# EryiXie/PlaneRecNet

Hardware: AMD Instinct MI355X
Metric: img/s fwd+bwd @480×640 ResNet101-DCN, 1/2/4/8 MI355X + roofline % (higher is better)
Workload: dtype f32 (tensors and accumulation fp32; plain GEMMs and the tap-walked 4x4/s2, 1x1/s2 and sub-pixel convolutions >= 300 tiles: 2xfp16-piece split MFMA, fp32 accumulate; fp32-only rate in fp32_only_run)

## Files before the change

planerecnet_amd/csrc/prn_dcn.hip:

```cpp
#include <stdlib.h>
#include "prn_common.h"

namespace {

struct Tap {
  int i00, i01, i10, i11;
  float w00, w01, w10, w11;
  float gy00, gy01, gy10, gy11, gx00, gx01, gx10, gx11;
  float mod;
  float sig;
  bool pass_y, pass_x;
};

struct OmView {
  const float* off; const float* msk;
  int64_t off_bs, msk_bs;
  float maxoff;
  int raw, pad;
};

__device__ __forceinline__ Tap make_tap(const OmView& v, int b, int k, int ho, int wo, int Ho, int Wo,
                                        int H, int W, int stride, bool need_grad) {
  Tap t;
  const size_t plane = (size_t)Ho * Wo, pix = (size_t)ho * Wo + wo;
  const float* ob = v.off + (size_t)b * v.off_bs;
  const float ry = ob[(2 * k) * plane + pix], rx = ob[(2 * k + 1) * plane + pix];
  float dy = ry, dx = rx;
  t.pass_y = t.pass_x = true;
  if (v.raw) {
    const float maxoff = v.maxoff;
    const float rm = ob[(18 + k) * plane + pix];
    dy = fminf(fmaxf(ry, -maxoff), maxoff); dx = fminf(fmaxf(rx, -maxoff), maxoff);
    t.pass_y = (ry >= -maxoff) && (ry <= maxoff);
    t.pass_x = (rx >= -maxoff) && (rx <= maxoff);
    t.sig = 1.f / (1.f + expf(-rm));
    t.mod = 2.f * t.sig;
  } else {
    t.sig = 0.f;
    t.mod = v.msk ? v.msk[(size_t)b * v.msk_bs + (size_t)k * plane + pix] : 1.f;
  }
  const int ki = k / 3, kj = k - ki * 3;
  const float y = (float)(ho * stride - v.pad + ki) + dy, x = (float)(wo * stride - v.pad + kj) + dx;
  const bool inside = (y > -1.f) && (y < (float)H) && (x > -1.f) && (x < (float)W);
  const float fy = floorf(y), fx = floorf(x);
  const int y0 = (int)fy, x0 = (int)fx, y1 = y0 + 1, x1 = x0 + 1;
  const float ly = y - fy, lx = x - fx, hy = 1.f - ly, hx = 1.f - lx;
  const bool vy0 = inside && y0 >= 0, vy1 = inside && y1 <= H - 1, vx0 = x0 >= 0, vx1 = x1 <= W - 1;
  const bool v00 = vy0 && vx0, v01 = vy0 && vx1, v10 = vy1 && vx0, v11 = vy1 && vx1;
  t.i00 = v00 ? y0 * W + x0 : 0; t.i01 = v01 ? y0 * W + x1 : 0;
  t.i10 = v10 ? y1 * W + x0 : 0; t.i11 = v11 ? y1 * W + x1 : 0;
  t.w00 = v00 ? hy * hx : 0.f; t.w01 = v01 ? hy * lx : 0.f;
  t.w10 = v10 ? ly * hx : 0.f; t.w11 = v11 ? ly * lx : 0.f;
  if (need_grad) {
    t.gy00 = v00 ? -hx : 0.f; t.gy01 = v01 ? -lx : 0.f; t.gy10 = v10 ? hx : 0.f; t.gy11 = v11 ? lx : 0.f;
    t.gx00 = v00 ? -hy : 0.f; t.gx01 = v01 ? hy : 0.f; t.gx10 = v10 ? -ly : 0.f; t.gx11 = v11 ? ly : 0.f;
  }
  return t;
}

__global__ __launch_bounds__(256) void dcn_sample_kernel(const float* __restrict__ x, OmView om,
                                                         float* __restrict__ cols, int B, int C, int H, int W, int Ho,
                                                         int Wo, int stride) {
  const int64_t gid = (int64_t)blockIdx.x * blockDim.x + threadIdx.x;
  const int64_t plane = (int64_t)Ho * Wo;
  if (gid >= (int64_t)B * 9 * plane) return;
  const int pix = gid % plane, k = (gid / plane) % 9, b = gid / (9 * plane);
  const int ho = pix / Wo, wo = pix - ho * Wo;
  const Tap t = make_tap(om, b, k, ho, wo, Ho, Wo, H, W, stride, false);
  const int cper = (C + gridDim.y - 1) / gridDim.y;
  const int c0 = blockIdx.y * cper, c1 = min(C, c0 + cper);
  const size_t HW = (size_t)H * W;
  const float* xp = x + ((size_t)b * C + c0) * HW;
  float* cp = cols + (((size_t)b * C + c0) * 9 + k) * plane + pix;
  constexpr int UN = 8;
  int c = c0;
  for (; c + UN <= c1; c += UN) {
    float a00[UN], a01[UN], a10[UN], a11[UN];
#pragma unroll
    for (int u = 0; u < UN; ++u) {
      const float* q = xp + (size_t)u * HW;
      a00[u] = q[t.i00]; a01[u] = q[t.i01]; a10[u] = q[t.i10]; a11[u] = q[t.i11];
    }
    __builtin_amdgcn_sched_barrier(0);
#pragma unroll
    for (int u = 0; u < UN; ++u) cp[(size_t)u * 9 * plane] = t.mod * (t.w00 * a00[u] + t.w01 * a01[u] + t.w10 * a10[u] + t.w11 * a11[u]);
    xp += (size_t)UN * HW;
    cp += (size_t)UN * 9 * plane;
  }
  for (; c < c1; ++c) {
    const float v = t.w00 * xp[t.i00] + t.w01 * xp[t.i01] + t.w10 * xp[t.i10] + t.w11 * xp[t.i11];
    *cp = t.mod * v;
    xp += HW;
    cp += 9 * plane;
  }
}

__global__ __launch_bounds__(256) void dcn_dom_partial_kernel(const float* __restrict__ x, OmView om,
                                                              const float* __restrict__ dcols, float* __restrict__ part, int B,
                                                              int C, int H, int W, int Ho, int Wo, int stride) {
  const int64_t gid = (int64_t)blockIdx.x * blockDim.x + threadIdx.x;
  const int64_t plane = (int64_t)Ho * Wo;
  if (gid >= (int64_t)B * 9 * plane) return;
  const int pix = gid % plane, k = (gid / plane) % 9, b = gid / (9 * plane);
  const int ho = pix / Wo, wo = pix - ho * Wo;
  const Tap t = make_tap(om, b, k, ho, wo, Ho, Wo, H, W, stride, true);
  const int cper = (C + gridDim.y - 1) / gridDim.y;
  const int c0 = blockIdx.y * cper, c1 = min(C, c0 + cper);
  const size_t HW = (size_t)H * W;
  const float* xp = x + ((size_t)b * C + c0) * HW;
  const float* dp = dcols + (((size_t)b * C + c0) * 9 + k) * plane + pix;
  float gy = 0.f, gx = 0.f, gm = 0.f;
  constexpr int UN = 8;
  int c = c0;
  for (; c + UN <= c1; c += UN) {
    float g[UN], a00[UN], a01[UN], a10[UN], a11[UN];
#pragma unroll
    for (int u = 0; u < UN; ++u) {
      const float* q = xp + (size_t)u * HW;
      g[u] = dp[(size_t)u * 9 * plane];
      a00[u] = q[t.i00]; a01[u] = q[t.i01]; a10[u] = q[t.i10]; a11[u] = q[t.i11];
    }
    __builtin_amdgcn_sched_barrier(0);
#pragma unroll
    for (int u = 0; u < UN; ++u) {
      gm += g[u] * (t.w00 * a00[u] + t.w01 * a01[u] + t.w10 * a10[u] + t.w11 * a11[u]);
      gy += g[u] * (t.gy00 * a00[u] + t.gy01 * a01[u] + t.gy10 * a10[u] + t.gy11 * a11[u]);
      gx += g[u] * (t.gx00 * a00[u] + t.gx01 * a01[u] + t.gx10 * a10[u] + t.gx11 * a11[u]);
    }
    xp += (size_t)UN * HW;
    dp += (size_t)UN * 9 * plane;
  }
  for (; c < c1; ++c) {
    const float g = *dp;
    const float x00 = xp[t.i00], x01 = xp[t.i01], x10 = xp[t.i10], x11 = xp[t.i11];
    gm += g * (t.w00 * x00 + t.w01 * x01 + t.w10 * x10 + t.w11 * x11);
    gy += g * (t.gy00 * x00 + t.gy01 * x01 + t.gy10 * x10 + t.gy11 * x11);
    gx += g * (t.gx00 * x00 + t.gx01 * x01 + t.gx10 * x10 + t.gx11 * x11);
    xp += HW;
    dp += 9 * plane;
  }
  float* ob = part + ((size_t)blockIdx.y * B + b) * 27 * plane + pix;
  ob[(2 * k) * plane] = t.pass_y ? gy * t.mod : 0.f;
  ob[(2 * k + 1) * plane] = t.pass_x ? gx * t.mod : 0.f;
  ob[(18 + k) * plane] = om.raw ? gm * 2.f * t.sig * (1.f - t.sig) : gm;
}

__global__ void dcn_dom_final_kernel(const float* __restrict__ part, float* __restrict__ d_off, float* __restrict__ d_msk, int64_t n, int G,
                                     int plane) {
  const int64_t i = (int64_t)blockIdx.x * blockDim.x + threadIdx.x;
  if (i >= n) return;
  float s = 0.f;
  for (int g = 0; g < G; ++g) s += part[(size_t)g * n + i];
  if (d_msk == nullptr) { d_off[i] = s; return; }
  const int64_t b = i / (27 * (int64_t)plane), r = i - b * 27 * (int64_t)plane;
  if (r < 18 * (int64_t)plane) d_off[b * 18 * plane + r] = s;
  else d_msk[b * 9 * plane + (r - 18 * (int64_t)plane)] = s;
}

struct CsrEntry { int src; float w; };

__device__ __forceinline__ bool csr_before(const CsrEntry& a, const CsrEntry& b) {
  return a.src < b.src || (a.src == b.src && __float_as_uint(a.w) < __float_as_uint(b.w));
}
__device__ __forceinline__ void csr_sort_bin(CsrEntry* __restrict__ e, int n) {
  if (n <= 8) {
    unsigned long long k[8];
    const unsigned long long* __restrict__ q = reinterpret_cast<const unsigned long long*>(e);
#pragma unroll
    for (int i = 0; i < 8; ++i) {
      const unsigned long long v = i < n ? q[i] : ~0ull;
      k[i] = i < n ? ((v << 32) | (v >> 32)) : ~0ull;
    }
#define PRN_CSR_CX(I, J) { const unsigned long long lo = k[I] < k[J] ? k[I] : k[J], hi = k[I] < k[J] ? k[J] : k[I]; k[I] = lo; k[J] = hi; }
    PRN_CSR_CX(0, 2) PRN_CSR_CX(1, 3) PRN_CSR_CX(4, 6) PRN_CSR_CX(5, 7) PRN_CSR_CX(0, 4) PRN_CSR_CX(1, 5) PRN_CSR_CX(2, 6) PRN_CSR_CX(3, 7)
    PRN_CSR_CX(0, 1) PRN_CSR_CX(2, 3) PRN_CSR_CX(4, 5) PRN_CSR_CX(6, 7) PRN_CSR_CX(2, 4) PRN_CSR_CX(3, 5) PRN_CSR_CX(1, 4) PRN_CSR_CX(3, 6)
    PRN_CSR_CX(1, 2) PRN_CSR_CX(3, 4) PRN_CSR_CX(5, 6)
#undef PRN_CSR_CX
    unsigned long long* __restrict__ o = reinterpret_cast<unsigned long long*>(e);
#pragma unroll
    for (int i = 0; i < 8; ++i)
      if (i < n) o[i] = (k[i] << 32) | (k[i] >> 32);
    return;
  }
  for (int i = 1; i < n; ++i) {
    const CsrEntry v = e[i];
    int j = i - 1;
    while (j >= 0 && csr_before(v, e[j])) { e[j + 1] = e[j]; --j; }
    e[j + 1] = v;
  }
}
__global__ __launch_bounds__(256) void dcn_csr_sort_kernel(const int* __restrict__ starts, const int* __restrict__ counts, CsrEntry* __restrict__ entries, int nbins) {
  const int bin = blockIdx.x * 256 + threadIdx.x;
  if (bin < nbins && counts[bin] > 1) csr_sort_bin(entries + starts[bin], counts[bin]);
}

__global__ __launch_bounds__(256) void dcn_csr_count_kernel(OmView om, int* __restrict__ counts, int B, int H, int W,
                                                            int Ho, int Wo, int stride) {
  const int64_t gid = (int64_t)blockIdx.x * blockDim.x + threadIdx.x;
  const int plane = Ho * Wo;
  if (gid >= (int64_t)B * 9 * plane) return;
  const int pix = gid % plane, k = (gid / plane) % 9, b = gid / (9 * plane);
  const int ho = pix / Wo, wo = pix - ho * Wo;
  const Tap t = make_tap(om, b, k, ho, wo, Ho, Wo, H, W, stride, false);
  int* cb = counts + (size_t)(b * 9 + k) * H * W;
  if (t.w00 != 0.f) atomicAdd(cb + t.i00, 1);
  if (t.w01 != 0.f) atomicAdd(cb + t.i01, 1);
  if (t.w10 != 0.f) atomicAdd(cb + t.i10, 1);
  if (t.w11 != 0.f) atomicAdd(cb + t.i11, 1);
}

constexpr int SCAN_PER_THREAD = 8, SCAN_PER_BLOCK = 256 * SCAN_PER_THREAD;

__device__ __forceinline__ int block_sum_256(int v, int* sm) {
  for (int o = 32; o > 0; o >>= 1) v += __shfl_down(v, o);
  if ((threadIdx.x & 63) == 0) sm[threadIdx.x >> 6] = v;
  __syncthreads();
  const int t = sm[0] + sm[1] + sm[2] + sm[3];
  __syncthreads();
  return t;
}

__global__ __launch_bounds__(256) void dcn_csr_block_sums_kernel(const int* __restrict__ counts, int* __restrict__ bsum, int n) {
  __shared__ int sm[4];
  const int base = blockIdx.x * SCAN_PER_BLOCK + threadIdx.x * SCAN_PER_THREAD;
  int v = 0;
#pragma unroll
  for (int i = 0; i < SCAN_PER_THREAD; ++i) v += (base + i < n) ? counts[base + i] : 0;
  const int t = block_sum_256(v, sm);
  if (threadIdx.x == 0) bsum[blockIdx.x] = t;
}

__global__ __launch_bounds__(256) void dcn_csr_scan_kernel(int* __restrict__ counts, int* __restrict__ starts, const int* __restrict__ bsum,
                                                           int n) {
  __shared__ int sm[4];
  __shared__ int wave_tot[4];
  int pre = 0;
  for (int i = threadIdx.x; i < (int)blockIdx.x; i += 256) pre += bsum[i];
  pre = block_sum_256(pre, sm);
  const int base = blockIdx.x * SCAN_PER_BLOCK + threadIdx.x * SCAN_PER_THREAD;
  int c[SCAN_PER_THREAD], mine = 0;
#pragma unroll
  for (int i = 0; i < SCAN_PER_THREAD; ++i) { c[i] = (base + i < n) ? counts[base + i] : 0; mine += c[i]; }
  const int lane = threadIdx.x & 63, wv = threadIdx.x >> 6;
  int incl = mine;
  for (int o = 1; o < 64; o <<= 1) { const int u = __shfl_up(incl, o); if (lane >= o) incl += u; }
  if (lane == 63) wave_tot[wv] = incl;
  __syncthreads();
  int off = pre + incl - mine;
  for (int w = 0; w < wv; ++w) off += wave_tot[w];
#pragma unroll
  for (int i = 0; i < SCAN_PER_THREAD; ++i)
    if (base + i < n) { starts[base + i] = off; off += c[i]; counts[base + i] = 0; }
}

__global__ __launch_bounds__(256) void dcn_csr_fill_kernel(OmView om, const int* __restrict__ starts, int* __restrict__ cursor,
                                                           CsrEntry* __restrict__ entries, int B, int H, int W, int Ho, int Wo, int stride) {
  const int64_t gid = (int64_t)blockIdx.x * blockDim.x + threadIdx.x;
  const int plane = Ho * Wo;
  if (gid >= (int64_t)B * 9 * plane) return;
  const int pix = gid % plane, k = (gid / plane) % 9, b = gid / (9 * plane);
  const int ho = pix / Wo, wo = pix - ho * Wo;
  const Tap t = make_tap(om, b, k, ho, wo, Ho, Wo, H, W, stride, false);
  const size_t bb = (size_t)(b * 9 + k) * H * W;
  const int src = k * plane + pix;
  auto put = [&](int idx, float w) {
    if (w != 0.f) {
      const int pos = starts[bb + idx] + atomicAdd(cursor + bb + idx, 1);
      entries[pos] = CsrEntry{src, w * t.mod};
    }
  };
  put(t.i00, t.w00); put(t.i01, t.w01); put(t.i10, t.w10); put(t.i11, t.w11);
}

constexpr int CSR1_THREADS = 1024;
constexpr int CSR1_MAX_BINS = 15360;
static_assert(CSR1_MAX_BINS * 4 + (CSR1_THREADS / 64) * 4 <= 64 * 1024, "the bins and the scan scratch of one tap plane must fit gfx950's 64 KB of LDS per workgroup");

__global__ __launch_bounds__(CSR1_THREADS) void dcn_csr_build_kernel(OmView om, int* __restrict__ starts, int* __restrict__ counts,
                                                                      CsrEntry* __restrict__ entries, int H, int W, int Ho, int Wo, int stride) {
  extern __shared__ int csr_bins[];
  __shared__ int wave_tot[CSR1_THREADS / 64];
  const int bk = blockIdx.x, b = bk / 9, k = bk - b * 9;
  const int HW = H * W, plane = Ho * Wo, tid = threadIdx.x;
  for (int i = tid; i < HW; i += CSR1_THREADS) csr_bins[i] = 0;
  __syncthreads();
  for (int p = tid; p < plane; p += CSR1_THREADS) {
    const int ho = p / Wo, wo = p - ho * Wo;
    const Tap t = make_tap(om, b, k, ho, wo, Ho, Wo, H, W, stride, false);
    if (t.w00 != 0.f) atomicAdd(csr_bins + t.i00, 1);
    if (t.w01 != 0.f) atomicAdd(csr_bins + t.i01, 1);
    if (t.w10 != 0.f) atomicAdd(csr_bins + t.i10, 1);
    if (t.w11 != 0.f) atomicAdd(csr_bins + t.i11, 1);
  }
  __syncthreads();
  const int per = (HW + CSR1_THREADS - 1) / CSR1_THREADS;
  const int b0 = tid * per, b1 = min(HW, b0 + per);
  int mine = 0;
  for (int i = b0; i < b1; ++i) mine += csr_bins[i];
  const int lane = tid & 63, wv = tid >> 6;
  int incl = mine;
  for (int o = 1; o < 64; o <<= 1) { const int u = __shfl_up(incl, o); if (lane >= o) incl += u; }
  if (lane == 63) wave_tot[wv] = incl;
  __syncthreads();
  int off = incl - mine;
  for (int w = 0; w < wv; ++w) off += wave_tot[w];
  const int seg = bk * 4 * plane;
  const size_t gb = (size_t)bk * HW;
  for (int i = b0; i < b1; ++i) {
    const int c = csr_bins[i];
    starts[gb + i] = seg + off;
    counts[gb + i] = c;
    csr_bins[i] = off;
    off += c;
  }
  __syncthreads();
  for (int p = tid; p < plane; p += CSR1_THREADS) {
    const int ho = p / Wo, wo = p - ho * Wo;
    const Tap t = make_tap(om, b, k, ho, wo, Ho, Wo, H, W, stride, false);
    const int src = k * plane + p;
    if (t.w00 != 0.f) entries[seg + atomicAdd(csr_bins + t.i00, 1)] = CsrEntry{src, t.w00 * t.mod};
    if (t.w01 != 0.f) entries[seg + atomicAdd(csr_bins + t.i01, 1)] = CsrEntry{src, t.w01 * t.mod};
    if (t.w10 != 0.f) entries[seg + atomicAdd(csr_bins + t.i10, 1)] = CsrEntry{src, t.w10 * t.mod};
    if (t.w11 != 0.f) entries[seg + atomicAdd(csr_bins + t.i11, 1)] = CsrEntry{src, t.w11 * t.mod};
  }
  __syncthreads();
  for (int i = b0; i < b1; ++i) {
    const int beg = i > 0 ? csr_bins[i - 1] : 0, n = csr_bins[i] - beg;
    if (n > 1) csr_sort_bin(entries + seg + beg, n);
  }
}

template <int CH>
__global__ __launch_bounds__(256) void dcn_dx_gather_kernel(const float* __restrict__ dcols, const int* __restrict__ starts,
                                                            const int* __restrict__ counts, const CsrEntry* __restrict__ entries,
                                                            float* __restrict__ dx, int C, int HW, int plane) {
  const int q = blockIdx.x * 256 + threadIdx.x;
  if (q >= HW) return;
  const int b = blockIdx.z, c0 = blockIdx.y * CH;
  const size_t cstride = (size_t)9 * plane;
  const float* __restrict__ dp = dcols + ((size_t)b * C + c0) * cstride;
  float acc[CH];
#pragma unroll
  for (int cc = 0; cc < CH; ++cc) acc[cc] = 0.f;
  int st[9], cn[9];
#pragma unroll
  for (int k = 0; k < 9; ++k) {
    const size_t bin = (size_t)(b * 9 + k) * HW + q;
    st[k] = starts[bin];
    cn[k] = counts[bin];
  }
#pragma unroll
  for (int k = 0; k < 9; ++k) {
    const int s = st[k], n = cn[k];
    CsrEntry nxt;
    nxt.src = 0; nxt.w = 0.f;
    if (n > 0) nxt = entries[s];
    for (int e = s; e < s + n; ++e) {
      const CsrEntry en = nxt;
      if (e + 1 < s + n) nxt = entries[e + 1];
#pragma unroll
      for (int cc = 0; cc < CH; ++cc) acc[cc] += en.w * dp[cc * cstride + en.src];
    }
  }
  float* out = dx + ((size_t)b * C + c0) * HW + q;
#pragma unroll
  for (int cc = 0; cc < CH; ++cc)
    if (c0 + cc < C) out[(size_t)cc * HW] = acc[cc];
}

}

static int channel_groups(int C, int64_t threads) {
  static const int forced = prn_env_int("PRN_DCN_GROUPS", 0);
  int g = forced > 0 ? forced : (int)(1 + (256 * 8 * 256) / (threads > 0 ? threads : 1));
  if (g > 16) g = 16;
  if (g > C) g = C;
  while (g < C && C % g) ++g;
  return g < 1 ? 1 : g;
}

namespace {
OmView raw_view(const float* om, int Ho, int Wo, float max_offset) {
  OmView v;
  v.off = om; v.msk = nullptr; v.off_bs = v.msk_bs = (int64_t)27 * Ho * Wo; v.maxoff = max_offset; v.raw = 1; v.pad = 1;
  return v;
}
OmView desc_view(const prn_dcn_desc* d, const float* offset, const float* mask) {
  if (d->raw) { OmView v = raw_view(offset, d->Ho, d->Wo, d->max_offset); v.pad = d->pad; return v; }
  OmView v;
  v.off = offset; v.msk = mask; v.off_bs = (int64_t)18 * d->Ho * d->Wo; v.msk_bs = (int64_t)9 * d->Ho * d->Wo; v.maxoff = 0.f; v.raw = 0; v.pad = d->pad;
  return v;
}
}

extern "C" int prn_dcn_sample(const float* x, const float* om, float* cols, int B, int C, int H, int W, int Ho, int Wo,
                              int stride, float max_offset, void* stream) {
  PRN_REQUIRE(x && om && cols && B > 0 && C > 0 && H > 0 && W > 0 && Ho > 0 && Wo > 0, "prn_dcn_sample: bad arguments");
  PRN_REQUIRE(Ho == (H + 2 - 3) / stride + 1 && Wo == (W + 2 - 3) / stride + 1, "prn_dcn_sample: output size mismatch");
  const int64_t n = (int64_t)B * 9 * Ho * Wo;
  hipLaunchKernelGGL(dcn_sample_kernel, dim3(cdiv(n, 256), channel_groups(C, n)), dim3(256), 0, (hipStream_t)stream, x, raw_view(om, Ho, Wo, max_offset),
                     cols, B, C, H, W, Ho, Wo, stride);
  PRN_CHECK_LAUNCH("prn_dcn_sample");
  return 0;
}

namespace {
struct BwdWs { int64_t part, counts, starts, bsum, entries, total; int nbins, nblocks; };
BwdWs bwd_ws_layout(int B, int C, int H, int W, int Ho, int Wo) {
  auto up = [](int64_t v) { return (v + 255) / 256 * 256; };
  BwdWs l;
  l.nbins = B * 9 * H * W;
  l.nblocks = cdiv(l.nbins, SCAN_PER_BLOCK);
  l.part = 0;
  l.counts = up((int64_t)channel_groups(C, (int64_t)B * 9 * Ho * Wo) * B * 27 * Ho * Wo * 4);
  l.starts = l.counts + up((int64_t)l.nbins * 4);
  l.bsum = l.starts + up((int64_t)l.nbins * 4);
  l.entries = l.bsum + up((int64_t)l.nblocks * 4);
  l.total = l.entries + (int64_t)B * 9 * Ho * Wo * 4 * sizeof(CsrEntry);
  return l;
}

int launch_dom(const float* x, const OmView& v, const float* dcols, float* d_off, float* d_msk, char* wsb, const BwdWs& l, int B, int C, int H, int W,
               int Ho, int Wo, int stride, hipStream_t st) {
  const int64_t n = (int64_t)B * 9 * Ho * Wo;
  const int G = channel_groups(C, n);
  hipLaunchKernelGGL(dcn_dom_partial_kernel, dim3(cdiv(n, 256), G), dim3(256), 0, st, x, v, dcols, (float*)(wsb + l.part), B, C, H, W, Ho, Wo, stride);
  PRN_CHECK_LAUNCH("dcn d_om partial");
  const int64_t nom = (int64_t)B * 27 * Ho * Wo;
  hipLaunchKernelGGL(dcn_dom_final_kernel, dim3(cdiv(nom, 256)), dim3(256), 0, st, (const float*)(wsb + l.part), d_off, d_msk, nom, G, Ho * Wo);
  PRN_CHECK_LAUNCH("dcn d_om final");
  return 0;
}

int launch_dx(const OmView& v, const float* dcols, float* dx, char* wsb, const BwdWs& l, int B, int C, int H, int W, int Ho, int Wo, int stride,
              hipStream_t st) {
  const int64_t n = (int64_t)B * 9 * Ho * Wo;
  int* counts = (int*)(wsb + l.counts);
  int* starts = (int*)(wsb + l.starts);
  int* bsum = (int*)(wsb + l.bsum);
  CsrEntry* entries = (CsrEntry*)(wsb + l.entries);
  static const int one = prn_env_int("PRN_DCN_CSR1", 1);
  if (one && H * W <= CSR1_MAX_BINS) {
    hipLaunchKernelGGL(dcn_csr_build_kernel, dim3(B * 9), dim3(CSR1_THREADS), (size_t)H * W * sizeof(int), st, v, starts, counts, entries, H, W, Ho, Wo, stride);
  } else {
    if (hipMemsetAsync(counts, 0, (size_t)l.nbins * 4, st) != hipSuccess) { prn_set_error("dcn d-input: memset failed"); return 1; }
    hipLaunchKernelGGL(dcn_csr_count_kernel, dim3(cdiv(n, 256)), dim3(256), 0, st, v, counts, B, H, W, Ho, Wo, stride);
    hipLaunchKernelGGL(dcn_csr_block_sums_kernel, dim3(l.nblocks), dim3(256), 0, st, (const int*)counts, bsum, l.nbins);
    hipLaunchKernelGGL(dcn_csr_scan_kernel, dim3(l.nblocks), dim3(256), 0, st, counts, starts, (const int*)bsum, l.nbins);
    hipLaunchKernelGGL(dcn_csr_fill_kernel, dim3(cdiv(n, 256)), dim3(256), 0, st, v, (const int*)starts, counts, entries, B, H, W, Ho, Wo, stride);
    hipLaunchKernelGGL(dcn_csr_sort_kernel, dim3(cdiv(l.nbins, 256)), dim3(256), 0, st, (const int*)starts, (const int*)counts, entries, (int)l.nbins);
  }
  PRN_CHECK_LAUNCH("dcn d-input csr");
  const int HW = H * W;
  const int64_t blocks8 = (int64_t)cdiv(HW, 256) * cdiv(C, 8) * B;
  if (blocks8 >= 1024)
    hipLaunchKernelGGL((dcn_dx_gather_kernel<8>), dim3(cdiv(HW, 256), cdiv(C, 8), B), dim3(256), 0, st, dcols, (const int*)starts, (const int*)counts,
                       (const CsrEntry*)entries, dx, C, HW, Ho * Wo);
  else
    hipLaunchKernelGGL((dcn_dx_gather_kernel<4>), dim3(cdiv(HW, 256), cdiv(C, 4), B), dim3(256), 0, st, dcols, (const int*)starts, (const int*)counts,
                       (const CsrEntry*)entries, dx, C, HW, Ho * Wo);
  PRN_CHECK_LAUNCH("dcn d-input gather");
  return 0;
}
}

extern "C" int64_t prn_dcn_sample_bwd_ws_bytes(int B, int C, int H, int W, int Ho, int Wo) {
  if (B <= 0 || C <= 0 || H <= 0 || W <= 0 || Ho <= 0 || Wo <= 0 || (int64_t)B * 9 * H * W >= (1LL << 31)) return -1;
  return bwd_ws_layout(B, C, H, W, Ho, Wo).total;
}

extern "C" int prn_dcn_sample_bwd(const float* x, const float* om, const float* dcols, float* dx, float* d_om, void* ws,
                                  int B, int C, int H, int W, int Ho, int Wo, int stride, float max_offset, void* stream) {
  PRN_REQUIRE(x && om && dcols && dx && d_om && ws && B > 0 && C > 0, "prn_dcn_sample_bwd: bad arguments");
  PRN_REQUIRE((int64_t)B * 9 * H * W < (1LL << 31) && (int64_t)B * 36 * Ho * Wo < (1LL << 31), "prn_dcn_sample_bwd: map too large");
  hipStream_t st = (hipStream_t)stream;
  const BwdWs l = bwd_ws_layout(B, C, H, W, Ho, Wo);
  const OmView v = raw_view(om, Ho, Wo, max_offset);
  if (int e = launch_dom(x, v, dcols, d_om, nullptr, (char*)ws, l, B, C, H, W, Ho, Wo, stride, st)) return e;
  return launch_dx(v, dcols, dx, (char*)ws, l, B, C, H, W, Ho, Wo, stride, st);
}

namespace {
struct DataWs { int64_t dcols, gemm, rest, total; prn_conv_desc g; };
int data_ws_layout(const prn_dcn_desc* d, DataWs& l) {
  auto up = [](int64_t v) { return (v + 255) / 256 * 256; };
  prn_conv_desc& g = l.g;
  g.B = d->B; g.C = d->M; g.H = d->Ho; g.W = d->Wo; g.M = d->C * 9; g.KH = g.KW = 1; g.stride = 1; g.pad = 0; g.Ho = d->Ho; g.Wo = d->Wo;
  g.in_mode = PRN_IN_ZERO; g.dil = 1; g.epilogue = PRN_EPI_NONE; g.ystride = 0; g.yH = g.yW = 0; g.reserved = 0;
  g.opts = d->opts;
  const int64_t gb = prn_conv2d_fwd_ws_bytes(&g);
  if (gb < 0) return 2;
  if ((int64_t)d->B * 9 * d->H * d->W >= (1LL << 31) || (int64_t)d->B * 36 * d->Ho * d->Wo >= (1LL << 31)) { prn_set_error("prn_dcnv2_bwd: map too large"); return 2; }
  l.dcols = 0;
  l.gemm = up((int64_t)d->B * d->C * 9 * d->Ho * d->Wo * 4);
  l.rest = l.gemm + up(gb);
  l.total = l.rest + bwd_ws_layout(d->B, d->C, d->H, d->W, d->Ho, d->Wo).total;
  return 0;
}
int check_dcn_desc(const prn_dcn_desc* d, const char* who) {
  PRN_REQUIRE(d != nullptr && d->B > 0 && d->C > 0 && d->H > 0 && d->W > 0 && d->M > 0 && d->Ho > 0 && d->Wo > 0 && d->stride > 0 && d->pad >= 0,
              "%s: bad descriptor", who);
  PRN_REQUIRE(d->Ho == (d->H + 2 * d->pad - 3) / d->stride + 1 && d->Wo == (d->W + 2 * d->pad - 3) / d->stride + 1, "%s: output size mismatch", who);
  return 0;
}
}

extern "C" int64_t prn_dcnv2_bwd_ws_bytes(const prn_dcn_desc* d) {
  if (check_dcn_desc(d, "prn_dcnv2_bwd_ws_bytes")) return -1;
  DataWs l;
  if (data_ws_layout(d, l)) return -1;
  return l.total;
}

extern "C" int prn_dcnv2_bwd_input(const prn_dcn_desc* d, const float* dy, const float* wt, const void* wt_images, const float* offset, const float* mask,
                                   float* dx, void* ws, void* stream) {
  return prn_dcnv2_bwd_input_phase(d, dy, wt, wt_images, offset, mask, dx, ws, stream, 0);
}

extern "C" int prn_dcnv2_bwd_input_phase(const prn_dcn_desc* d, const float* dy, const float* wt, const void* wt_images, const float* offset, const float* mask,
                                         float* dx, void* ws, void* stream, int phase) {
  if (int e = check_dcn_desc(d, "prn_dcnv2_bwd_input")) return e;
  PRN_REQUIRE(dy && wt && offset && ws, "prn_dcnv2_bwd_input: null tensor");
  PRN_REQUIRE(phase >= 0 && phase <= 3, "prn_dcnv2_bwd_input: bad phase");
  DataWs l;
  if (int e = data_ws_layout(d, l)) return e;
  char* wsb = (char*)ws;
  if (phase <= 2)
    if (int e = prn_conv2d_fwd_counted(&l.g, dy, wt, wt_images, nullptr, nullptr, (float*)(wsb + l.dcols), wsb + l.gemm, nullptr, stream, phase)) return e;
  if (dx == nullptr || phase == 1 || phase == 2) return 0;
  const BwdWs bl = bwd_ws_layout(d->B, d->C, d->H, d->W, d->Ho, d->Wo);
  return launch_dx(desc_view(d, offset, mask), (const float*)(wsb + l.dcols), dx, wsb + l.rest, bl, d->B, d->C, d->H, d->W, d->Ho, d->Wo, d->stride,
                   (hipStream_t)stream);
}

extern "C" int prn_dcnv2_bwd_offset_mask(const prn_dcn_desc* d, const float* x, const float* offset, const float* mask, float* d_offset, float* d_mask,
                                         void* ws, void* stream) {
  if (int e = check_dcn_desc(d, "prn_dcnv2_bwd_offset_mask")) return e;
  PRN_REQUIRE(x && offset && d_offset && ws, "prn_dcnv2_bwd_offset_mask: null tensor");
  PRN_REQUIRE(d->raw || d_mask != nullptr, "prn_dcnv2_bwd_offset_mask: d_mask required unless the descriptor is raw (then d_offset is the [B,27,Ho,Wo] gradient)");
  DataWs l;
  if (int e = data_ws_layout(d, l)) return e;
  char* wsb = (char*)ws;
  const BwdWs bl = bwd_ws_layout(d->B, d->C, d->H, d->W, d->Ho, d->Wo);
  return launch_dom(x, desc_view(d, offset, mask), (const float*)(wsb + l.dcols), d_offset, d->raw ? nullptr : d_mask, wsb + l.rest, bl, d->B, d->C, d->H,
                    d->W, d->Ho, d->Wo, d->stride, (hipStream_t)stream);
}
```

Baseline: 188.5.

## Use channel-innermost column layout for DCNv2 backward gather and offset-gradient kernels

Recasts the DCNv2 backward column GEMM so the gradient columns come out as [B*P, 9, C], with channels innermost. This needs transposes of dy, the weights and x. New kernels then read those columns with vectorized float4 channel loads: a CSR gather for dx, and an offset/mask gradient kernel that uses wave shuffles and so no longer needs the partial-sum buffer and final reduction pass. The aim is to replace strided, uncoalesced column accesses with contiguous ones. The cost is extra transpose passes and more workspace, and the path is on by default behind an env switch.

After: 186.2. 0.988x the previous value.

```diff
diff --git a/planerecnet_amd/csrc/prn_dcn.hip b/planerecnet_amd/csrc/prn_dcn.hip
--- a/planerecnet_amd/csrc/prn_dcn.hip
+++ b/planerecnet_amd/csrc/prn_dcn.hip
@@ -368,6 +368,180 @@
     if (c0 + cc < C) out[(size_t)cc * HW] = acc[cc];
 }
 
+
+
+__global__ __launch_bounds__(256) void dcn_transpose_kernel(const float* __restrict__ in, float* __restrict__ out, int R, int Cn, int64_t irs, int64_t ors,
+                                                            int64_t izs, int64_t ozs) {
+  __shared__ float tile[32][33];
+  const int tx = threadIdx.x & 31, ty = threadIdx.x >> 5;
+  const int c0 = blockIdx.x * 32, r0 = blockIdx.y * 32;
+  const float* ip = in + (size_t)blockIdx.z * izs;
+  float* op = out + (size_t)blockIdx.z * ozs;
+#pragma unroll
+  for (int i = 0; i < 4; ++i) {
+    const int r = r0 + ty + 8 * i, c = c0 + tx;
+    if (r < R && c < Cn) tile[ty + 8 * i][tx] = ip[(size_t)r * irs + c];
+  }
+  __syncthreads();
+#pragma unroll
+  for (int i = 0; i < 4; ++i) {
+    const int c = c0 + ty + 8 * i, r = r0 + tx;
+    if (r < R && c < Cn) op[(size_t)c * ors + r] = tile[tx][ty + 8 * i];
+  }
+}
+
+template <bool VEC>
+__device__ __forceinline__ float4 load4(const float* __restrict__ v, int c, int C) {
+  if constexpr (VEC) {
+    return c < C ? *reinterpret_cast<const float4*>(v + c) : make_float4(0.f, 0.f, 0.f, 0.f);
+  } else {
+    float4 r;
+    r.x = c < C ? v[c] : 0.f; r.y = c + 1 < C ? v[c + 1] : 0.f; r.z = c + 2 < C ? v[c + 2] : 0.f; r.w = c + 3 < C ? v[c + 3] : 0.f;
+    return r;
+  }
+}
+
+constexpr int DXQ = 16;
+template <int GS, bool VEC>
+__global__ __launch_bounds__(DXQ * GS) void dcn_dx_cl_kernel(const float* __restrict__ G, const int* __restrict__ starts, const int* __restrict__ counts,
+                                                              const CsrEntry* __restrict__ entries, float* __restrict__ dx, int C, int HW, int plane) {
+  __shared__ float tile[4 * GS][DXQ + 1];
+  const int tid = threadIdx.x, grp = tid / GS, gl = tid % GS, lane = tid & 63, gbase = lane - gl;
+  const int b = blockIdx.z, cbase = blockIdx.y * 4 * GS, c = cbase + 4 * gl;
+  const int q = blockIdx.x * DXQ + grp;
+  const bool live = q < HW;
+  const float* __restrict__ Gb = G + (size_t)b * plane * 9 * C;
+  int st = 0, cn = 0;
+  if (live && gl < 9) {
+    const size_t bin = (size_t)(b * 9 + gl) * HW + q;
+    st = starts[bin]; cn = counts[bin];
+  }
+  int pre[10];
+  pre[0] = 0;
+#pragma unroll
+  for (int k = 0; k < 9; ++k) pre[k + 1] = pre[k] + __shfl(cn, gbase + k);
+  int stk[9];
+#pragma unroll
+  for (int k = 0; k < 9; ++k) stk[k] = __shfl(st, gbase + k);
+  const int T = pre[9];
+  float4 acc = make_float4(0.f, 0.f, 0.f, 0.f);
+  for (int t0 = 0; __any(t0 < T); t0 += GS) {
+    const int t = t0 + gl;
+    int off = 0;
+    float wgt = 0.f;
+    if (t < T) {
+      int k = 0;
+#pragma unroll
+      for (int j = 1; j < 9; ++j) k += (t >= pre[j]) ? 1 : 0;
+      int s = 0, p0 = 0;
+#pragma unroll
+      for (int j = 0; j < 9; ++j) { s = (j == k) ? stk[j] : s; p0 = (j == k) ? pre[j] : p0; }
+      const CsrEntry en = entries[s + (t - p0)];
+      off = ((en.src - k * plane) * 9 + k) * C;
+      wgt = en.w;
+    }
+    const int nround = min(GS, T - t0);
+    constexpr int UN = 8;
+    for (int e = 0; __any(e < nround); e += UN) {
+      float4 g[UN];
+      float w[UN];
+#pragma unroll
+      for (int u = 0; u < UN; ++u) {
+        const int o = __shfl(off, gbase + ((e + u) & (GS - 1)));
+        const float ww = __shfl(wgt, gbase + ((e + u) & (GS - 1)));
+        w[u] = (e + u < nround) ? ww : 0.f;
+        g[u] = load4<VEC>(Gb + ((e + u < nround) ? o : 0), c, C);
+      }
+      __builtin_amdgcn_sched_barrier(0);
+#pragma unroll
+      for (int u = 0; u < UN; ++u) { acc.x += w[u] * g[u].x; acc.y += w[u] * g[u].y; acc.z += w[u] * g[u].z; acc.w += w[u] * g[u].w; }
+    }
+  }
+  tile[4 * gl + 0][grp] = acc.x; tile[4 * gl + 1][grp] = acc.y; tile[4 * gl + 2][grp] = acc.z; tile[4 * gl + 3][grp] = acc.w;
+  __syncthreads();
+  const int q0 = blockIdx.x * DXQ;
+#pragma unroll
+  for (int i = 0; i < 4; ++i) {
+    const int idx = tid + i * DXQ * GS, cc = idx / DXQ, qi = idx % DXQ;
+    if (cbase + cc < C && q0 + qi < HW) dx[((size_t)b * C + cbase + cc) * HW + q0 + qi] = tile[cc][qi];
+  }
+}
+
+template <int GS, bool VEC>
+__global__ __launch_bounds__(256) void dcn_dom_cl_kernel(const float* __restrict__ xT, OmView om, const float* __restrict__ G, float* __restrict__ d_off,
+                                                         float* __restrict__ d_msk, int B, int C, int H, int W, int Ho, int Wo, int stride) {
+  const int tid = threadIdx.x, gl = tid % GS, lane = tid & 63, gbase = lane - gl;
+  const int plane = Ho * Wo;
+  const int64_t n = (int64_t)blockIdx.x * (256 / GS) + tid / GS;
+  const bool live = n < (int64_t)B * plane;
+  const int b = live ? (int)(n / plane) : 0, p = live ? (int)(n - (int64_t)b * plane) : 0;
+  const int ho = p / Wo, wo = p - ho * Wo;
+  const int myk = gl < 9 ? gl : 8;
+  const Tap t = make_tap(om, b, myk, ho, wo, Ho, Wo, H, W, stride, true);
+  const int j00 = (t.gy00 != 0.f || t.gx00 != 0.f) ? t.i00 * C : -1, j01 = (t.gy01 != 0.f || t.gx01 != 0.f) ? t.i01 * C : -1;
+  const int j10 = (t.gy10 != 0.f || t.gx10 != 0.f) ? t.i10 * C : -1, j11 = (t.gy11 != 0.f || t.gx11 != 0.f) ? t.i11 * C : -1;
+  const float* __restrict__ xb = xT + (size_t)b * H * W * C;
+  const float* __restrict__ gp = G + ((size_t)b * plane + p) * 9 * C;
+  float S0 = 0.f, S1 = 0.f, S2 = 0.f, S3 = 0.f;
+  constexpr int UT = 3;
+  for (int kb = 0; kb < 9; kb += UT) {
+    int o[UT][4];
+    float a[UT][4];
+#pragma unroll
+    for (int u = 0; u < UT; ++u) {
+      o[u][0] = __shfl(j00, gbase + kb + u); o[u][1] = __shfl(j01, gbase + kb + u);
+      o[u][2] = __shfl(j10, gbase + kb + u); o[u][3] = __shfl(j11, gbase + kb + u);
+      a[u][0] = a[u][1] = a[u][2] = a[u][3] = 0.f;
+    }
+    for (int c = 4 * gl; __any(c < C); c += 4 * GS) {
+      float4 g[UT], xv[UT][4];
+#pragma unroll
+      for (int u = 0; u < UT; ++u) {
+        g[u] = load4<VEC>(gp + (size_t)(kb + u) * C, c, C);
+#pragma unroll
+        for (int j = 0; j < 4; ++j) xv[u][j] = load4<VEC>(xb + (o[u][j] < 0 ? 0 : o[u][j]), c, C);
+      }
+      __builtin_amdgcn_sched_barrier(0);
+#pragma unroll
+      for (int u = 0; u < UT; ++u)
+#pragma unroll
+        for (int j = 0; j < 4; ++j) {
+          const float d = g[u].x * xv[u][j].x + g[u].y * xv[u][j].y + g[u].z * xv[u][j].z + g[u].w * xv[u][j].w;
+          a[u][j] += o[u][j] < 0 ? 0.f : d;
+        }
+    }
+#pragma unroll
+    for (int u = 0; u < UT; ++u) {
+      const bool h1 = (gl & 1) != 0, h2 = (gl & 2) != 0;
+      float k0 = h1 ? a[u][2] : a[u][0], k1 = h1 ? a[u][3] : a[u][1];
+      const float s0 = h1 ? a[u][0] : a[u][2], s1 = h1 ? a[u][1] : a[u][3];
+      k0 += __shfl_xor(s0, 1); k1 += __shfl_xor(s1, 1);
+      float kk = h2 ? k1 : k0;
+      const float ss = h2 ? k0 : k1;
+      kk += __shfl_xor(ss, 2);
+#pragma unroll
+      for (int w = 4; w < GS; w <<= 1) kk += __shfl_xor(kk, w);
+      const float r0 = __shfl(kk, gbase + 0), r1 = __shfl(kk, gbase + 2), r2 = __shfl(kk, gbase + 1), r3 = __shfl(kk, gbase + 3);
+      if (gl == kb + u) { S0 = r0; S1 = r1; S2 = r2; S3 = r3; }
+    }
+  }
+  if (!live || gl >= 9) return;
+  const float gm = t.w00 * S0 + t.w01 * S1 + t.w10 * S2 + t.w11 * S3;
+  const float gy = t.gy00 * S0 + t.gy01 * S1 + t.gy10 * S2 + t.gy11 * S3;
+  const float gx = t.gx00 * S0 + t.gx01 * S1 + t.gx10 * S2 + t.gx11 * S3;
+  const float vy = t.pass_y ? gy * t.mod : 0.f, vx = t.pass_x ? gx * t.mod : 0.f;
+  const float vm = om.raw ? gm * 2.f * t.sig * (1.f - t.sig) : gm;
+  const int k = gl;
+  if (d_msk == nullptr) {
+    float* ob = d_off + (size_t)b * 27 * plane + p;
+    ob[(size_t)(2 * k) * plane] = vy; ob[(size_t)(2 * k + 1) * plane] = vx; ob[(size_t)(18 + k) * plane] = vm;
+  } else {
+    float* ob = d_off + (size_t)b * 18 * plane + p;
+    ob[(size_t)(2 * k) * plane] = vy; ob[(size_t)(2 * k + 1) * plane] = vx;
+    d_msk[((size_t)b * 9 + k) * plane + p] = vm;
+  }
+}
+
 }
 
 static int channel_groups(int C, int64_t threads) {
@@ -406,13 +580,17 @@
 
 namespace {
 struct BwdWs { int64_t part, counts, starts, bsum, entries, total; int nbins, nblocks; };
-BwdWs bwd_ws_layout(int B, int C, int H, int W, int Ho, int Wo) {
+bool bwd_cl() {
+  static const int on = prn_env_int("PRN_DCN_BWD_CL", 1);
+  return on != 0;
+}
+BwdWs bwd_ws_layout(int B, int C, int H, int W, int Ho, int Wo, bool with_part = true) {
   auto up = [](int64_t v) { return (v + 255) / 256 * 256; };
   BwdWs l;
   l.nbins = B * 9 * H * W;
   l.nblocks = cdiv(l.nbins, SCAN_PER_BLOCK);
   l.part = 0;
-  l.counts = up((int64_t)channel_groups(C, (int64_t)B * 9 * Ho * Wo) * B * 27 * Ho * Wo * 4);
+  l.counts = with_part ? up((int64_t)channel_groups(C, (int64_t)B * 9 * Ho * Wo) * B * 27 * Ho * Wo * 4) : 0;
   l.starts = l.counts + up((int64_t)l.nbins * 4);
   l.bsum = l.starts + up((int64_t)l.nbins * 4);
   l.entries = l.bsum + up((int64_t)l.nblocks * 4);
@@ -433,7 +611,7 @@
 }
 
 int launch_dx(const OmView& v, const float* dcols, float* dx, char* wsb, const BwdWs& l, int B, int C, int H, int W, int Ho, int Wo, int stride,
-              hipStream_t st) {
+              hipStream_t st, bool cl = false) {
   const int64_t n = (int64_t)B * 9 * Ho * Wo;
   int* counts = (int*)(wsb + l.counts);
   int* starts = (int*)(wsb + l.starts);
@@ -452,6 +630,17 @@
   }
   PRN_CHECK_LAUNCH("dcn d-input csr");
   const int HW = H * W;
+  if (cl) {
+    const int lanes = cdiv(C < 256 ? C : 256, 4), gs = lanes <= 16 ? 16 : (lanes <= 32 ? 32 : 64);
+    const dim3 grid(cdiv(HW, DXQ), cdiv(C, 4 * gs), B);
+#define PRN_DX_CL(GS_, VEC_) hipLaunchKernelGGL((dcn_dx_cl_kernel<GS_, VEC_>), grid, dim3(DXQ * GS_), 0, st, dcols, (const int*)starts, (const int*)counts, \
+                                               (const CsrEntry*)entries, dx, C, HW, Ho * Wo)
+    if ((C & 3) == 0) { if (gs == 16) PRN_DX_CL(16, true); else if (gs == 32) PRN_DX_CL(32, true); else PRN_DX_CL(64, true); }
+    else { if (gs == 16) PRN_DX_CL(16, false); else if (gs == 32) PRN_DX_CL(32, false); else PRN_DX_CL(64, false); }
+#undef PRN_DX_CL
+    PRN_CHECK_LAUNCH("dcn d-input gather (channel-innermost)");
+    return 0;
+  }
   const int64_t blocks8 = (int64_t)cdiv(HW, 256) * cdiv(C, 8) * B;
   if (blocks8 >= 1024)
     hipLaunchKernelGGL((dcn_dx_gather_kernel<8>), dim3(cdiv(HW, 256), cdiv(C, 8), B), dim3(256), 0, st, dcols, (const int*)starts, (const int*)counts,
@@ -462,6 +651,25 @@
   PRN_CHECK_LAUNCH("dcn d-input gather");
   return 0;
 }
+
+int launch_transpose(const float* in, float* out, int R, int Cn, int64_t irs, int64_t ors, int64_t izs, int64_t ozs, int Z, hipStream_t st) {
+  hipLaunchKernelGGL(dcn_transpose_kernel, dim3(cdiv(Cn, 32), cdiv(R, 32), Z), dim3(256), 0, st, in, out, R, Cn, irs, ors, izs, ozs);
+  PRN_CHECK_LAUNCH("dcn transpose");
+  return 0;
+}
+
+int launch_dom_cl(const float* x, float* xT, const OmView& v, const float* G, float* d_off, float* d_msk, int B, int C, int H, int W, int Ho, int Wo, int stride,
+                  hipStream_t st) {
+  if (int e = launch_transpose(x, xT, C, H * W, (int64_t)H * W, C, (int64_t)C * H * W, (int64_t)C * H * W, B, st)) return e;
+  const int lanes = cdiv(C < 256 ? C : 256, 4), gs = lanes <= 16 ? 16 : (lanes <= 32 ? 32 : 64);
+  const dim3 grid(cdiv((int64_t)B * Ho * Wo, 256 / gs));
+#define PRN_DOM_CL(GS_, VEC_) hipLaunchKernelGGL((dcn_dom_cl_kernel<GS_, VEC_>), grid, dim3(256), 0, st, (const float*)xT, v, G, d_off, d_msk, B, C, H, W, Ho, Wo, stride)
+  if ((C & 3) == 0) { if (gs == 16) PRN_DOM_CL(16, true); else if (gs == 32) PRN_DOM_CL(32, true); else PRN_DOM_CL(64, true); }
+  else { if (gs == 16) PRN_DOM_CL(16, false); else if (gs == 32) PRN_DOM_CL(32, false); else PRN_DOM_CL(64, false); }
+#undef PRN_DOM_CL
+  PRN_CHECK_LAUNCH("dcn d_om (channel-innermost)");
+  return 0;
+}
 }
 
 extern "C" int64_t prn_dcn_sample_bwd_ws_bytes(int B, int C, int H, int W, int Ho, int Wo) {
@@ -481,11 +689,18 @@
 }
 
 namespace {
-struct DataWs { int64_t dcols, gemm, rest, total; prn_conv_desc g; };
+struct DataWs { int64_t dcols, gemm, dyT, wp, rest, xT, total; bool cl; prn_conv_desc g; };
 int data_ws_layout(const prn_dcn_desc* d, DataWs& l) {
   auto up = [](int64_t v) { return (v + 255) / 256 * 256; };
   prn_conv_desc& g = l.g;
-  g.B = d->B; g.C = d->M; g.H = d->Ho; g.W = d->Wo; g.M = d->C * 9; g.KH = g.KW = 1; g.stride = 1; g.pad = 0; g.Ho = d->Ho; g.Wo = d->Wo;
+  l.cl = bwd_cl();
+  const int64_t P = (int64_t)d->Ho * d->Wo;
+  if (l.cl) {
+    if ((int64_t)d->B * P >= (1LL << 29)) { prn_set_error("prn_dcnv2_bwd: map too large"); return 2; }
+    g.B = 1; g.C = d->M; g.H = 9; g.W = d->C; g.M = (int)(d->B * P); g.KH = g.KW = 1; g.stride = 1; g.pad = 0; g.Ho = 9; g.Wo = d->C;
+  } else {
+    g.B = d->B; g.C = d->M; g.H = d->Ho; g.W = d->Wo; g.M = d->C * 9; g.KH = g.KW = 1; g.stride = 1; g.pad = 0; g.Ho = d->Ho; g.Wo = d->Wo;
+  }
   g.in_mode = PRN_IN_ZERO; g.dil = 1; g.epilogue = PRN_EPI_NONE; g.ystride = 0; g.yH = g.yW = 0; g.reserved = 0;
   g.opts = d->opts;
   const int64_t gb = prn_conv2d_fwd_ws_bytes(&g);
@@ -493,8 +708,11 @@
   if ((int64_t)d->B * 9 * d->H * d->W >= (1LL << 31) || (int64_t)d->B * 36 * d->Ho * d->Wo >= (1LL << 31)) { prn_set_error("prn_dcnv2_bwd: map too large"); return 2; }
   l.dcols = 0;
   l.gemm = up((int64_t)d->B * d->C * 9 * d->Ho * d->Wo * 4);
-  l.rest = l.gemm + up(gb);
-  l.total = l.rest + bwd_ws_layout(d->B, d->C, d->H, d->W, d->Ho, d->Wo).total;
+  l.dyT = l.gemm + up(gb);
+  l.wp = l.dyT + (l.cl ? up((int64_t)d->B * P * d->M * 4) : 0);
+  l.rest = l.wp + (l.cl ? up((int64_t)d->M * 9 * d->C * 4) : 0);
+  l.xT = l.rest + up(bwd_ws_layout(d->B, d->C, d->H, d->W, d->Ho, d->Wo, !l.cl).total);
+  l.total = l.xT + (l.cl ? up((int64_t)d->B * d->C * d->H * d->W * 4) : 0);
   return 0;
 }
 int check_dcn_desc(const prn_dcn_desc* d, const char* who) {
@@ -525,12 +743,24 @@
   DataWs l;
   if (int e = data_ws_layout(d, l)) return e;
   char* wsb = (char*)ws;
-  if (phase <= 2)
-    if (int e = prn_conv2d_fwd_counted(&l.g, dy, wt, wt_images, nullptr, nullptr, (float*)(wsb + l.dcols), wsb + l.gemm, nullptr, stream, phase)) return e;
+  if (phase <= 2) {
+    if (l.cl) {
+      const int P = d->Ho * d->Wo, C = d->C, M = d->M;
+      float* dyT = (float*)(wsb + l.dyT);
+      float* wp = (float*)(wsb + l.wp);
+      if (phase != 2) {
+        if (int e = launch_transpose(dy, dyT, M, P, P, M, (int64_t)M * P, (int64_t)M * P, d->B, (hipStream_t)stream)) return e;
+        if (int e = launch_transpose(wt, wp, C, M, (int64_t)9 * M, (int64_t)9 * C, M, C, 9, (hipStream_t)stream)) return e;
+      }
+      if (int e = prn_conv2d_fwd_counted(&l.g, wp, dyT, nullptr, nullptr, nullptr, (float*)(wsb + l.dcols), wsb + l.gemm, nullptr, stream, phase)) return e;
+    } else {
+      if (int e = prn_conv2d_fwd_counted(&l.g, dy, wt, wt_images, nullptr, nullptr, (float*)(wsb + l.dcols), wsb + l.gemm, nullptr, stream, phase)) return e;
+    }
+  }
   if (dx == nullptr || phase == 1 || phase == 2) return 0;
-  const BwdWs bl = bwd_ws_layout(d->B, d->C, d->H, d->W, d->Ho, d->Wo);
+  const BwdWs bl = bwd_ws_layout(d->B, d->C, d->H, d->W, d->Ho, d->Wo, !l.cl);
   return launch_dx(desc_view(d, offset, mask), (const float*)(wsb + l.dcols), dx, wsb + l.rest, bl, d->B, d->C, d->H, d->W, d->Ho, d->Wo, d->stride,
-                   (hipStream_t)stream);
+                   (hipStream_t)stream, l.cl);
 }
 
 extern "C" int prn_dcnv2_bwd_offset_mask(const prn_dcn_desc* d, const float* x, const float* offset, const float* mask, float* d_offset, float* d_mask,
@@ -541,6 +771,9 @@
   DataWs l;
   if (int e = data_ws_layout(d, l)) return e;
   char* wsb = (char*)ws;
+  if (l.cl)
+    return launch_dom_cl(x, (float*)(wsb + l.xT), desc_view(d, offset, mask), (const float*)(wsb + l.dcols), d_offset, d->raw ? nullptr : d_mask, d->B, d->C,
+                         d->H, d->W, d->Ho, d->Wo, d->stride, (hipStream_t)stream);
   const BwdWs bl = bwd_ws_layout(d->B, d->C, d->H, d->W, d->Ho, d->Wo);
   return launch_dom(x, desc_view(d, offset, mask), (const float*)(wsb + l.dcols), d_offset, d->raw ? nullptr : d_mask, wsb + l.rest, bl, d->B, d->C, d->H,
                     d->W, d->Ho, d->Wo, d->stride, (hipStream_t)stream);
```
